# lucidrains/magvit2-pytorch

Measured on NVIDIA H100. Metric: video-frames/sec tokenize+decode, 17x128x128 bf16, higher is better.
Workload: dtype bf16

## Files before the change

### magvit2_pytorch_b200/csrc/tc_common.cuh

```cuda
#pragma once
#include "common.cuh"
#include <cuda.h>
#include <mutex>

namespace mv2 {


__device__ __forceinline__ uint32_t smem_u32(const void* p) { return (uint32_t)__cvta_generic_to_shared(p); }

__device__ __forceinline__ void mbar_init(uint32_t bar, uint32_t count) {
  asm volatile("mbarrier.init.shared::cta.b64 [%0], %1;" ::"r"(bar), "r"(count));
}
__device__ __forceinline__ void mbar_expect_tx(uint32_t bar, uint32_t bytes) {
  asm volatile("mbarrier.arrive.expect_tx.shared::cta.b64 _, [%0], %1;" ::"r"(bar), "r"(bytes) : "memory");
}
__device__ __forceinline__ void mbar_wait(uint32_t bar, uint32_t parity) {
  asm volatile(
      "{\n\t"
      ".reg .pred P1;\n\t"
      "WAIT_LOOP:\n\t"
      "mbarrier.try_wait.parity.shared::cta.b64 P1, [%0], %1, 0x989680;\n\t"
      "@P1 bra DONE;\n\t"
      "bra WAIT_LOOP;\n\t"
      "DONE:\n\t"
// ... 36 lines not shown

template <int N> __device__ __forceinline__ void setmaxnreg_dec() { asm volatile("setmaxnreg.dec.sync.aligned.u32 %0;" ::"n"(N)); }
template <int N> __device__ __forceinline__ void setmaxnreg_inc() { asm volatile("setmaxnreg.inc.sync.aligned.u32 %0;" ::"n"(N)); }
template <int N> __device__ __forceinline__ void wgmma_bf16(float (&d)[N / 2], uint64_t da, uint64_t db, uint32_t scale_d);
template <> __device__ __forceinline__ void wgmma_bf16<8>(float (&d)[4], uint64_t da, uint64_t db, uint32_t scale_d) {
  asm volatile(
      "{\n\t.reg .pred p;\n\tsetp.ne.b32 p, %6, 0;\n\t"
      "wgmma.mma_async.sync.aligned.m64n8k16.f32.bf16.bf16 {%0, %1, %2, %3}, %4, %5, p, 1, 1, 0, 0;\n\t}"
      : "+f"(d[0]), "+f"(d[1]), "+f"(d[2]), "+f"(d[3])
      : "l"(da), "l"(db), "r"(scale_d));
}
template <> __device__ __forceinline__ void wgmma_bf16<16>(float (&d)[8], uint64_t da, uint64_t db, uint32_t scale_d) {
  asm volatile(
      "{\n\t.reg .pred p;\n\tsetp.ne.b32 p, %10, 0;\n\t"
      "wgmma.mma_async.sync.aligned.m64n16k16.f32.bf16.bf16 {%0, %1, %2, %3, %4, %5, %6, %7}, %8, %9, p, 1, 1, 0, 0;\n\t}"
      : "+f"(d[0]), "+f"(d[1]), "+f"(d[2]), "+f"(d[3]), "+f"(d[4]), "+f"(d[5]), "+f"(d[6]), "+f"(d[7])
      : "l"(da), "l"(db), "r"(scale_d));
}
template <> __device__ __forceinline__ void wgmma_bf16<32>(float (&d)[16], uint64_t da, uint64_t db, uint32_t scale_d) {
  asm volatile(
      "{\n\t.reg .pred p;\n\tsetp.ne.b32 p, %18, 0;\n\t"
      "wgmma.mma_async.sync.aligned.m64n32k16.f32.bf16.bf16 {%0, %1, %2, %3, %4, %5, %6, %7, %8, %9, %10, %11, %12, %13, %14, %15}, %16, %17, p, 1, 1, 0, 0;\n\t}"
      : "+f"(d[0]), "+f"(d[1]), "+f"(d[2]), "+f"(d[3]), "+f"(d[4]), "+f"(d[5]), "+f"(d[6]), "+f"(d[7]), "+f"(d[8]), "+f"(d[9]), "+f"(d[10]), "+f"(d[11]), "+f"(d[12]), "+f"(d[13]), "+f"(d[14]), "+f"(d[15])
      : "l"(da), "l"(db), "r"(scale_d));
}
template <> __device__ __forceinline__ void wgmma_bf16<64>(float (&d)[32], uint64_t da, uint64_t db, uint32_t scale_d) {
  asm volatile(
      "{\n\t.reg .pred p;\n\tsetp.ne.b32 p, %34, 0;\n\t"
      "wgmma.mma_async.sync.aligned.m64n64k16.f32.bf16.bf16 {%0, %1, %2, %3, %4, %5, %6, %7, %8, %9, %10, %11, %12, %13, %14, %15, %16, %17, %18, %19, %20, %21, %22, %23, %24, %25, %26, %27, %28, %29, %30, %31}, %32, %33, p, 1, 1, 0, 0;\n\t}"
      : "+f"(d[0]), "+f"(d[1]), "+f"(d[2]), "+f"(d[3]), "+f"(d[4]), "+f"(d[5]), "+f"(d[6]), "+f"(d[7]), "+f"(d[8]), "+f"(d[9]), "+f"(d[10]), "+f"(d[11]), "+f"(d[12]), "+f"(d[13]), "+f"(d[14]), "+f"(d[15]), "+f"(d[16]), "+f"(d[17]), "+f"(d[18]), "+f"(d[19]), "+f"(d[20]), "+f"(d[21]), "+f"(d[22]), "+f"(d[23]), "+f"(d[24]), "+f"(d[25]), "+f"(d[26]), "+f"(d[27]), "+f"(d[28]), "+f"(d[29]), "+f"(d[30]), "+f"(d[31])
      : "l"(da), "l"(db), "r"(scale_d));
}
template <> __device__ __forceinline__ void wgmma_bf16<128>(float (&d)[64], uint64_t da, uint64_t db, uint32_t scale_d) {
  asm volatile(
      "{\n\t.reg .pred p;\n\tsetp.ne.b32 p, %66, 0;\n\t"
      "wgmma.mma_async.sync.aligned.m64n128k16.f32.bf16.bf16 {%0, %1, %2, %3, %4, %5, %6, %7, %8, %9, %10, %11, %12, %13, %14, %15, %16, %17, %18, %19, %20, %21, %22, %23, %24, %25, %26, %27, %28, %29, %30, %31, %32, %33, %34, %35, %36, %37, %38, %39, %40, %41, %42, %43, %44, %45, %46, %47, %48, %49, %50, %51, %52, %53, %54, %55, %56, %57, %58, %59, %60, %61, %62, %63}, %64, %65, p, 1, 1, 0, 0;\n\t}"
      : "+f"(d[0]), "+f"(d[1]), "+f"(d[2]), "+f"(d[3]), "+f"(d[4]), "+f"(d[5]), "+f"(d[6]), "+f"(d[7]), "+f"(d[8]), "+f"(d[9]), "+f"(d[10]), "+f"(d[11]), "+f"(d[12]), "+f"(d[13]), "+f"(d[14]), "+f"(d[15]), "+f"(d[16]), "+f"(d[17]), "+f"(d[18]), "+f"(d[19]), "+f"(d[20]), "+f"(d[21]), "+f"(d[22]), "+f"(d[23]), "+f"(d[24]), "+f"(d[25]), "+f"(d[26]), "+f"(d[27]), "+f"(d[28]), "+f"(d[29]), "+f"(d[30]), "+f"(d[31]), "+f"(d[32]), "+f"(d[33]), "+f"(d[34]), "+f"(d[35]), "+f"(d[36]), "+f"(d[37]), "+f"(d[38]), "+f"(d[39]), "+f"(d[40]), "+f"(d[41]), "+f"(d[42]), "+f"(d[43]), "+f"(d[44]), "+f"(d[45]), "+f"(d[46]), "+f"(d[47]), "+f"(d[48]), "+f"(d[49]), "+f"(d[50]), "+f"(d[51]), "+f"(d[52]), "+f"(d[53]), "+f"(d[54]), "+f"(d[55]), "+f"(d[56]), "+f"(d[57]), "+f"(d[58]), "+f"(d[59]), "+f"(d[60]), "+f"(d[61]), "+f"(d[62]), "+f"(d[63])
      : "l"(da), "l"(db), "r"(scale_d));
}

__host__ __device__ __forceinline__ uint64_t gmma_desc_hi(uint32_t sbo, uint32_t row_bytes) {
  const uint64_t layout = row_bytes == 128 ? 1 : (row_bytes == 64 ? 2 : 3);
  return ((uint64_t)1 << 16) | ((uint64_t)(sbo >> 4) << 32) | (layout << 62);
}
__device__ __forceinline__ uint32_t desc_lo(uint32_t saddr) { return (saddr & 0x3FFFF) >> 4; }

template <int N> __device__ __forceinline__ void stage_acc(const float (&d)[N / 2], float* stg, int t) {
  const int r = 16 * (t >> 5) + ((t & 31) >> 2), c = 2 * (t & 3);
#pragma unroll
  for (int j = 0; j < N / 8; ++j) {
    *reinterpret_cast<float2*>(stg + r * (N + 4) + 8 * j + c) = make_float2(d[4 * j], d[4 * j + 1]);
    *reinterpret_cast<float2*>(stg + (r + 8) * (N + 4) + 8 * j + c) = make_float2(d[4 * j + 2], d[4 * j + 3]);
  }
}
__device__ __forceinline__ void load_row32(const float* src, int ncols, uint32_t (&r)[32]) {
#pragma unroll
  for (int g = 0; g < 8; ++g) {
    if (g * 4 >= ncols) break;
    const float4 v = *reinterpret_cast<const float4*>(src + 4 * g);
    r[4 * g] = __float_as_uint(v.x); r[4 * g + 1] = __float_as_uint(v.y);
    r[4 * g + 2] = __float_as_uint(v.z); r[4 * g + 3] = __float_as_uint(v.w);
  }
}
__device__ __forceinline__ void named_bar_sync(uint32_t id, uint32_t nthreads) {
  asm volatile("bar.sync %0, %1;" ::"r"(id), "r"(nthreads) : "memory");
}
__device__ __forceinline__ void mbar_arrive(uint32_t bar) {
  asm volatile("mbarrier.arrive.shared::cta.b64 _, [%0];" ::"r"(bar) : "memory");
}

__device__ __forceinline__ uint32_t pack_bf16x2(float a, float b) {
  __nv_bfloat162 v = __floats2bfloat162_rn(a, b);
  return *reinterpret_cast<uint32_t*>(&v);
}



struct TcEpi {
  const float* bias;
  const __nv_bfloat16* res;
  __nv_bfloat16* y;
  int act, shuffle, mode;
  int Co;
  int To, Ho, Wo;
  int out_cf;
  const float* oscale;
};

__device__ __forceinline__ void store8_bf16(__nv_bfloat16* dst, const float (&v)[8]) {
  uint4 o;
  o.x = pack_bf16x2(v[0], v[1]); o.y = pack_bf16x2(v[2], v[3]);
  o.z = pack_bf16x2(v[4], v[5]); o.w = pack_bf16x2(v[6], v[7]);
  *reinterpret_cast<uint4*>(dst) = o;
}

enum { EPI_PLAIN = 0, EPI_GEGLU = 1, EPI_SHUFFLE = 2, EPI_RAGGED = 3, EPI_PLAIN_RES = 4, EPI_FUSED_RU = 5, EPI_SHUFFLE_ST = 6,
       EPI_DOWN_SPACE = 7 };

__device__ __forceinline__ float ex2_approx(float x) {
  float y;
  asm("ex2.approx.ftz.f32 %0, %1;" : "=f"(y) : "f"(x));
  return y;
}
__device__ __forceinline__ float rcp_approx(float x) {
  float y;
  asm("rcp.approx.ftz.f32 %0, %1;" : "=f"(y) : "f"(x));
// ... 189 lines not shown
```

### magvit2_pytorch_b200/csrc/tc_slab.cu

```cuda
#include "common.cuh"
#include "tc_common.cuh"
#include <cuda.h>
#include <algorithm>
#include <type_traits>
#include <mutex>
#include <map>
#include <vector>
#include <string.h>

namespace mv2 {

struct alignas(64) SlabParams {
  CUtensorMap amap;
  CUtensorMap hmap;
  CUtensorMap wmap;
  CUtensorMap wmap2;
  int kt, kh, kw, pt, ph, pw;
  int st;
  int hist_T;
  int Ci, kchunks, row_bytes;
  int B, T, H, W, Co;
  int mw, pitch, slab_h, slab_bytes, slab_stride;
  int bn, n_tiles_n, tiles_w, tiles_h, total_tiles;
  int slab_stages, w_stages;
  int tpw;
  TcEpi epi;
  CUtensorMap w1map;
  const float* bias1;
  const float* se_wk;
  float se_bk;
  float* se_ws;
  CUtensorMap amap_odd;
  int dn_e_off;
  int dn_aoff[6];
  int dn_lower;
  int h_stride;
  CUtensorMap ymap;
  CUtensorMap rmap;
};

__host__ __device__ constexpr bool slab_tma_epi(int mode) {
  return mode == EPI_PLAIN || mode == EPI_PLAIN_RES || mode == EPI_GEGLU || mode == EPI_DOWN_SPACE;
}
__host__ __device__ constexpr int slab_out_box_ch(int mode, int bn) {
  return (mode == EPI_GEGLU ? bn / 2 : bn) < 64 ? (mode == EPI_GEGLU ? bn / 2 : bn) : 64;
}

__host__ __device__ __forceinline__ void slab_frame_of(const SlabParams& p, int slot, int& b, int& t) {
  const int ptc = p.pt > 0 ? (p.pt + p.st - 1) / p.st : 0;
  const int n_cheap = ptc < p.T ? ptc : p.T, n_full = p.T - n_cheap;
  const int full_slots = p.B * n_full;
  if (slot < full_slots) { b = slot / n_full; t = n_cheap + slot - b * n_full; }
  else { const int r = slot - full_slots; const int level = r / p.B; b = r - level * p.B; t = n_cheap - 1 - level; }
}
__host__ __device__ __forceinline__ int slab_tile_of_cta(const SlabParams& p, int k, int cta, int grid) {
  const int tile = k * grid + ((k & 1) ? grid - 1 - cta : cta);
  return tile < p.total_tiles ? tile : -1;
}
__device__ __forceinline__ int slab_tile_of(const SlabParams& p, int k) { return slab_tile_of_cta(p, k, blockIdx.x, gridDim.x); }

struct TileCoord { int b, t, h0, w0, n0; };
__host__ __device__ __forceinline__ TileCoord decode_tile(const SlabParams& p, int tile) {
  TileCoord c;
  const int nt = tile % p.n_tiles_n; tile /= p.n_tiles_n;
  const int tw = tile % p.tiles_w; tile /= p.tiles_w;
  const int th = tile % p.tiles_h; tile /= p.tiles_h;
  slab_frame_of(p, tile, c.b, c.t);
  c.h0 = th * 16;
  c.w0 = tw * 8 * p.mw;
  c.n0 = nt * p.bn;
  return c;
}

struct SlabSmem { uint32_t sbias, stage0, lpart, accstg, hbuf, end, rbar, otile, rtile; };
__host__ __device__ __forceinline__ SlabSmem slab_smem_layout(const SlabParams& p, uint32_t bar0, bool fused) {
  SlabSmem m;
  m.sbias = (bar0 + 8 * (2 * p.slab_stages + 2 * p.w_stages) + 15) & ~15u;
  m.stage0 = m.sbias + (uint32_t)(p.n_tiles_n * p.bn) * 4 * (fused ? 3 : 1);
  m.lpart = m.stage0 + (fused ? 0 : 8 * 2048);
  m.accstg = m.lpart + (fused ? 2048 : 0);
  m.hbuf = m.accstg + 2u * p.mw * 64 * (p.bn + 4) * 4;
  if (fused) m.hbuf = (m.hbuf + 1023u) & ~1023u;
  m.end = m.hbuf + (fused ? (uint32_t)p.h_stride : 0);
  m.rbar = m.stage0;
  m.otile = (m.rbar + 32 + 1023u) & ~1023u;
  m.rtile = m.otile + 2u * p.mw * 64 * p.bn * 2;
  return m;
}

template <int MODE, int BN, int ACT, int MWMAX>
__device__ __forceinline__ void slab_epi_fragment(const SlabParams& p, const float (&acc)[MWMAX][BN / 2], const TileCoord& c,
                                                  const float* sbias, uint32_t ot, uint32_t rt, int wq, int lane, bool relu) {
  constexpr int OC = MODE == EPI_GEGLU ? BN / 2 : BN, CB = slab_out_box_ch(MODE, BN), NB = OC / CB;
  constexpr uint32_t RB = CB * 2, BOX = 64 * RB, SWZ = (RB / 16 - 1) << 4;
  const uint32_t m0 = 16 * wq + (lane >> 2), q4 = (lane & 3) * 4;
  auto at = [&](int j, int col, uint32_t m) {
    const uint32_t off = m * RB + (uint32_t)(col % CB) * 2 + q4;
    return (uint32_t)(j * NB + col / CB) * BOX + (off ^ ((off >> 3) & SWZ));
  };
  auto st32 = [](uint32_t a, uint32_t v) { asm volatile("st.shared.b32 [%0], %1;" ::"r"(a), "r"(v) : "memory"); };
  const float* os = (MODE == EPI_PLAIN || MODE == EPI_PLAIN_RES) && p.epi.oscale ? p.epi.oscale + (int64_t)c.b * p.Co : nullptr;
  const float rs = MODE == EPI_PLAIN_RES && p.epi.mode == 2 ? 0.70710678118654752440f : 1.f;
#pragma unroll
  for (int j = 0; j < MWMAX; ++j) {
    if (j >= p.mw) break;
    if (MODE == EPI_GEGLU) {
#pragma unroll
      for (int g = 0; g < BN / 16; ++g) {
        const int n = c.n0 + 16 * g + 2 * (lane & 3);
        const float2 bx = *reinterpret_cast<const float2*>(sbias + n), bg = *reinterpret_cast<const float2*>(sbias + n + 8);
#pragma unroll
        for (int hr = 0; hr < 2; ++hr) {
          const float* xv = &acc[j][8 * g + 2 * hr];
          const float* gv = &acc[j][8 * g + 4 + 2 * hr];
          const float v0 = gelu_fast(gv[0] + bg.x) * (xv[0] + bx.x);
          const float v1 = gelu_fast(gv[1] + bg.y) * (xv[1] + bx.y);
          st32(ot + at(j, 8 * g, m0 + 8 * hr), pack_bf16x2(v0, v1));
        }
      }
    } else {
#pragma unroll
      for (int g = 0; g < BN / 8; ++g) {
        const int col = 8 * g, n = c.n0 + col + 2 * (lane & 3);
        const float2 b = *reinterpret_cast<const float2*>(sbias + n);
        float o0 = 1.f, o1 = 1.f;
        if (os) { o0 = n < p.Co ? os[n] : 0.f; o1 = n + 1 < p.Co ? os[n + 1] : 0.f; }
#pragma unroll
        for (int hr = 0; hr < 2; ++hr) {
          float v0 = acc[j][4 * g + 2 * hr], v1 = acc[j][4 * g + 2 * hr + 1];
          if (os) { v0 *= o0; v1 *= o1; }
          v0 = act_ct<ACT>(v0 + b.x, relu);
          v1 = act_ct<ACT>(v1 + b.y, relu);
          const uint32_t a = at(j, col, m0 + 8 * hr);
          if (MODE == EPI_PLAIN_RES) {
            uint32_t r;
            asm volatile("ld.shared.b32 %0, [%1];" : "=r"(r) : "r"(rt + a) : "memory");
            v0 = (v0 + __uint_as_float(r << 16)) * rs;
            v1 = (v1 + __uint_as_float(r & 0xffff0000u)) * rs;
          }
          st32(ot + a, pack_bf16x2(v0, v1));
        }
      }
    }
  }
}

constexpr int SLAB_PRODUCER_REGS = 40, SLAB_CONSUMER_REGS = 232;
template <int MODE, int BN>
__global__ void __launch_bounds__(384, 1) tc_slab_kernel(const __grid_constant__ SlabParams p) {
  constexpr int MWMAX = BN >= 32 ? 128 / BN : 4;
  constexpr int KC1 = BN >= 64 ? BN / 64 : 1;
  extern __shared__ uint8_t smem_raw[];
  const uint32_t smem_base = (smem_u32(smem_raw) + 1023u) & ~1023u;
  const int warp = threadIdx.x >> 5, lane = threadIdx.x & 31;
  const uint32_t row_bytes = p.row_bytes;
  const uint32_t bk = row_bytes >> 1;
  const uint32_t w_tile = p.bn * row_bytes;
  const uint32_t w_bytes = w_tile * p.tpw;
  const uint32_t slab0 = smem_base;
  const uint32_t wst0 = smem_base + p.slab_stages * p.slab_stride;
  const uint32_t bar0 = wst0 + p.w_stages * w_bytes;
  const uint32_t slab_full = bar0, slab_empty = slab_full + 8 * p.slab_stages;
  const uint32_t w_full = slab_empty + 8 * p.slab_stages, w_empty = w_full + 8 * p.w_stages;
  const SlabSmem L = slab_smem_layout(p, bar0, MODE == EPI_FUSED_RU);
  auto gen = [&](uint32_t u) { return smem_raw + (u - smem_u32(smem_raw)); };
  float* sbias = reinterpret_cast<float*>(gen(L.sbias));
  const uint32_t nbias = (uint32_t)(p.n_tiles_n * p.bn);
  const uint32_t stage0 = L.stage0;

  if (threadIdx.x == 0) {
    for (int s = 0; s < p.slab_stages; ++s) { mbar_init(slab_full + 8 * s, 1); mbar_init(slab_empty + 8 * s, 8); }
    for (int s = 0; s < p.w_stages; ++s) { mbar_init(w_full + 8 * s, 1); mbar_init(w_empty + 8 * s, 8); }
    if (MODE == EPI_PLAIN_RES)
      for (int g = 0; g < 2; ++g) { mbar_init(L.rbar + 8 * g, 1); mbar_init(L.rbar + 16 + 8 * g, 4); }
    fence_barrier_init();
  }
  if (warp == 0 && lane == 0) {
    tma_prefetch_desc(&p.amap);
    if (MODE == EPI_DOWN_SPACE) tma_prefetch_desc(&p.amap_odd);
    else if (p.hist_T > 0) tma_prefetch_desc(&p.hmap);
  }
  if (warp == 2 && lane == 0) {
    tma_prefetch_desc(&p.wmap); tma_prefetch_desc(&p.wmap2);
    if (MODE == EPI_FUSED_RU) tma_prefetch_desc(&p.w1map);
  }
  if (slab_tma_epi(MODE) && warp == 1 && lane == 0) {
    tma_prefetch_desc(&p.ymap);
    if (MODE == EPI_PLAIN_RES) tma_prefetch_desc(&p.rmap);
  }
  if (warp >= 4) {
    const int nb = p.n_tiles_n * p.bn;
    for (int i = threadIdx.x - 128; i < nb; i += 256) sbias[i] = (p.epi.bias && i < p.Co) ? p.epi.bias[i] : 0.f;
    if (MODE == EPI_FUSED_RU)
      for (int i = threadIdx.x - 128; i < nb; i += 256) {
        sbias[nb + i] = (p.bias1 && i < p.Co) ? p.bias1[i] : 0.f;
        sbias[2 * nb + i] = i < p.Co ? p.se_wk[i] : 0.f;
      }
  }
  __syncthreads();
  pdl_wait();
  pdl_launch_dependents();

  const int taps2d = p.kh * p.kw;

// ... 57 lines not shown
      if (MODE == EPI_DOWN_SPACE) {
        if (lane == 0) {
          uint32_t s = 0, ph = 0;
          const int C2 = p.Ci;
          for (int tk = 0, tile; (tile = slab_tile_of(p, tk)) >= 0; ++tk) {
            const TileCoord c = decode_tile(p, tile);
            for (int kc = 0; kc < p.kchunks; ++kc)
              for (int tap = kc < p.dn_lower ? 1 : 0; tap < 6; tap += kc < p.dn_lower ? 2 : 1) {
                mbar_wait(w_empty + 8 * s, ph ^ 1);
                mbar_expect_tx(w_full + 8 * s, w_tile);
                tma_load_2d(wst0 + s * w_bytes, &p.wmap2, w_full + 8 * s, tap * C2 + kc * (int)bk, c.n0);
                if (++s == (uint32_t)p.w_stages) { s = 0; ph ^= 1; }
              }
          }
        }
      } else
      if (lane == 0) {
        uint32_t s = 0, ph = 0;
        for (int tk = 0, tile; (tile = slab_tile_of(p, tk)) >= 0; ++tk) {
          const TileCoord c = decode_tile(p, tile);
          const int dt0 = max(0, p.pt - c.t * p.st - p.hist_T);
          for (int dt = dt0; dt < p.kt; ++dt)
            for (int kc = 0; kc < p.kchunks; ++kc)
              for (int tp = 0; tp < taps2d; tp += p.tpw) {
                mbar_wait(w_empty + 8 * s, ph ^ 1);
                mbar_expect_tx(w_full + 8 * s, w_bytes);
                if (p.tpw == 1) tma_load_2d(wst0 + s * w_bytes, &p.wmap2, w_full + 8 * s, (dt * taps2d + tp) * p.Ci + kc * bk, c.n0);
                else tma_load_3d(wst0 + s * w_bytes, &p.wmap, w_full + 8 * s, kc * bk, c.n0, dt * taps2d + tp);
                if (++s == (uint32_t)p.w_stages) { s = 0; ph ^= 1; }
              }
          if (MODE == EPI_FUSED_RU)
            for (int kc2 = 0; kc2 < KC1; ++kc2) {
              mbar_wait(w_empty + 8 * s, ph ^ 1);
              mbar_expect_tx(w_full + 8 * s, w_tile);
              tma_load_2d(wst0 + s * w_bytes, &p.w1map, w_full + 8 * s, kc2 * (int)bk, 0);
              if (++s == (uint32_t)p.w_stages) { s = 0; ph ^= 1; }
            }
        }
      }
    }
  } else {
    setmaxnreg_inc<SLAB_CONSUMER_REGS>();
    const int wg = (warp - 4) >> 2, wq = warp & 3, tid = threadIdx.x & 127;
    const int sub = 2 * wg + (wq & 1), half = wq >> 1, ew = sub + 4 * half;
    const int row = sub * 32 + lane;
    const int lh = row >> 3, lw = row & 7;
    float* stg = reinterpret_cast<float*>(gen(L.accstg)) + (size_t)wg * p.mw * 64 * (BN + 4);
    const uint32_t wg_bar = 5 + wg;
    const uint32_t sbo = (uint32_t)p.pitch * row_bytes;
    const uint64_t a_hi = gmma_desc_hi(sbo, row_bytes);
    const uint64_t b_hi = gmma_desc_hi(8 * row_bytes, row_bytes);
    const bool k4 = bk == 64;
    const uint32_t a_row = row_bytes >> 4;
    const uint32_t a_wg = (uint32_t)wg * 8 * (sbo >> 4);
    const uint32_t a_next_dh = (uint32_t)(p.pitch - p.kw + 1) * a_row;
    const uint32_t a_mtile = 8 * a_row;
    const uint32_t w_tile16 = w_tile >> 4, w_stage16 = w_bytes >> 4;
    const uint32_t b_lo0 = desc_lo(wst0);
    uint32_t s_idx = 0, s_par = 0;
    uint32_t w_idx = 0, w_par = 0, b_lo = b_lo0;
    uint32_t ecount = 0;
    uint32_t r_par = 0;
    float acc[MWMAX][BN / 2];
    auto mainloop = [&](const TileCoord& c, auto mw_c, auto k4_c) {
      constexpr int MW = decltype(mw_c)::value;
      constexpr bool K4 = decltype(k4_c)::value;
      constexpr uint32_t NONE = ~0u;
      uint32_t accum = 0, pend_w = NONE, pend_s = NONE;
      auto release_pending = [&]() {
        __syncwarp();
        if (lane == 0) {
          if (pend_w != NONE) mbar_arrive(w_empty + 8 * pend_w);
          if (pend_s != NONE) mbar_arrive(slab_empty + 8 * pend_s);
        }
      };
      auto retire_previous = [&](uint32_t w_last, uint32_t s_last) {
        wgmma_wait<1>();
        release_pending();
        pend_w = w_last; pend_s = s_last;
      };
      auto next_w_stage = [&]() {
        if (++w_idx == (uint32_t)p.w_stages) { w_idx = 0; w_par ^= 1; b_lo = b_lo0; } else { b_lo += w_stage16; }
      };
      if (MODE == EPI_DOWN_SPACE) {
        for (int kc = 0; kc < p.kchunks; ++kc) {
          mbar_wait(slab_full + 8 * s_idx, s_par);
          const uint32_t a_base = desc_lo(slab0 + s_idx * p.slab_stride) + a_wg;
          const int t0 = kc < p.dn_lower ? 1 : 0, tstep = kc < p.dn_lower ? 2 : 1;
          for (int tap = t0; tap < 6; tap += tstep) {
            mbar_wait(w_full + 8 * w_idx, w_par);
            wgmma_fence();
            const uint64_t bd = b_hi | (uint64_t)b_lo;
#pragma unroll
            for (int j = 0; j < MW; ++j) {
              const uint64_t ad = a_hi | (uint64_t)(a_base + (uint32_t)p.dn_aoff[tap] + j * a_mtile);
              wgmma_bf16<BN>(acc[j], ad, bd, accum);
              wgmma_bf16<BN>(acc[j], ad + 2, bd + 2, 1u);
              wgmma_bf16<BN>(acc[j], ad + 4, bd + 4, 1u);
              wgmma_bf16<BN>(acc[j], ad + 6, bd + 6, 1u);
            }
            wgmma_commit();
            retire_previous(w_idx, tap + tstep >= 6 ? s_idx : NONE);
            accum = 1;
            next_w_stage();
          }
          if (++s_idx == (uint32_t)p.slab_stages) { s_idx = 0; s_par ^= 1; }
        }
      } else {
        const int dt0 = max(0, p.pt - c.t * p.st - p.hist_T);
        for (int dt = dt0; dt < p.kt; ++dt)
          for (int kc = 0; kc < p.kchunks; ++kc) {
            mbar_wait(slab_full + 8 * s_idx, s_par);
            uint32_t a_lo = desc_lo(slab0 + s_idx * p.slab_stride) + a_wg;
            int dw = 0;
            for (int tp0 = 0; tp0 < taps2d; tp0 += p.tpw) {
              mbar_wait(w_full + 8 * w_idx, w_par);
              const bool slab_last = tp0 + p.tpw >= taps2d;
              uint32_t b_cur = b_lo;
              for (int u = 0; u < p.tpw; ++u) {
                wgmma_fence();
                const uint64_t bd = b_hi | (uint64_t)b_cur;
#pragma unroll
                for (int j = 0; j < MW; ++j) {
                  const uint64_t ad = a_hi | (uint64_t)(a_lo + j * a_mtile);
                  wgmma_bf16<BN>(acc[j], ad, bd, accum);
                  wgmma_bf16<BN>(acc[j], ad + 2, bd + 2, 1u);
                  if (K4) {
                    wgmma_bf16<BN>(acc[j], ad + 4, bd + 4, 1u);
                    wgmma_bf16<BN>(acc[j], ad + 6, bd + 6, 1u);
                  }
                }
                wgmma_commit();
                const bool w_last = u == p.tpw - 1;
                retire_previous(w_last ? w_idx : NONE, w_last && slab_last ? s_idx : NONE);
                accum = 1;
                b_cur += w_tile16;
                if (++dw == p.kw) { dw = 0; a_lo += a_next_dh; } else { a_lo += a_row; }
              }
              next_w_stage();
            }
            if (++s_idx == (uint32_t)p.slab_stages) { s_idx = 0; s_par ^= 1; }
          }
      }
      wgmma_wait<0>();
      release_pending();
    };
    auto mainloop_k = [&](const TileCoord& c, auto mw_c) {
      if (MODE != EPI_FUSED_RU && MODE != EPI_DOWN_SPACE && !k4) mainloop(c, mw_c, std::false_type());
      else mainloop(c, mw_c, std::true_type());
    };
    for (int tk = 0, tile; (tile = slab_tile_of(p, tk)) >= 0; ++tk) {
      const TileCoord c = decode_tile(p, tile);
      if (MWMAX >= 4 && p.mw == 4) mainloop_k(c, std::integral_constant<int, (MWMAX >= 4 ? 4 : 1)>());
      else if (MWMAX >= 2 && p.mw == 2) mainloop_k(c, std::integral_constant<int, (MWMAX >= 2 ? 2 : 1)>());
      else mainloop_k(c, std::integral_constant<int, 1>());
      if (slab_tma_epi(MODE)) {
        constexpr int CB = slab_out_box_ch(MODE, BN), NB = (MODE == EPI_GEGLU ? BN / 2 : BN) / CB;
        constexpr uint32_t BOX = 64 * CB * 2;
        const uint32_t ot = L.otile + (uint32_t)(wg * p.mw * NB) * BOX, rt = L.rtile + (uint32_t)(wg * p.mw) * 64 * BN * 2;
        if (tid == 0) bulk_wait_read_all();
        named_bar_sync(wg_bar, 128);
        if (MODE == EPI_PLAIN_RES) mbar_wait(L.rbar + 8 * wg, r_par);
        const int act = p.epi.act;
        if (MODE == EPI_GEGLU || act == MV2_ACT_NONE)
          slab_epi_fragment<MODE, BN, MV2_ACT_NONE>(p, acc, c, sbias, ot, rt, wq, lane, false);
        else if (act == MV2_ACT_ELU) slab_epi_fragment<MODE, BN, MV2_ACT_ELU>(p, acc, c, sbias, ot, rt, wq, lane, false);
        else if (act == MV2_ACT_SILU) slab_epi_fragment<MODE, BN, MV2_ACT_SILU>(p, acc, c, sbias, ot, rt, wq, lane, false);
        else slab_epi_fragment<MODE, BN, MV2_ACT_LEAKY_RELU>(p, acc, c, sbias, ot, rt, wq, lane, act == MV2_ACT_RELU);
        if (MODE == EPI_PLAIN_RES) {
          __syncwarp();
          if (lane == 0) mbar_arrive(L.rbar + 16 + 8 * wg);
          r_par ^= 1;
        }
        fence_proxy_async();
        named_bar_sync(wg_bar, 128);
        if (tid == 0) {
          const int oc0 = MODE == EPI_GEGLU ? c.n0 / 2 : c.n0, oco = MODE == EPI_GEGLU ? p.Co / 2 : p.Co;
          const int h = c.h0 + 8 * wg;
          for (int j = 0; j < p.mw; ++j)
            for (int b = 0; b < NB; ++b)
              if (h < p.H && c.w0 + 8 * j < p.W && oc0 + b * CB < oco)
                tma_store_5d(&p.ymap, ot + (uint32_t)(j * NB + b) * BOX, oc0 + b * CB, c.w0 + 8 * j, h, c.t, c.b);
          bulk_commit();
        }
        continue;
      }
      named_bar_sync(wg_bar, 128);
#pragma unroll
      for (int j = 0; j < MWMAX; ++j) {
        if (j >= p.mw) break;
        stage_acc<BN>(acc[j], stg + j * 64 * (BN + 4), tid);
      }
      named_bar_sync(wg_bar, 128);
      const int h = c.h0 + lh;
      if (MODE == EPI_FUSED_RU) {
        const float* sb1 = sbias + nbias;
        const float* swk = sbias + 2 * nbias;
        float* lpart = reinterpret_cast<float*>(gen(L.lpart));
        const int64_t kstride = (int64_t)p.W * p.Co;
        const uint32_t wsw = (lane >> 1) & 3;
        const int rl = lane >> 2, piece = lane & 3;
        const int h20 = c.h0 + sub * 4;
        const int recs_per_frame = p.tiles_h * p.tiles_w * 4;
        float* rec = p.se_ws + ((int64_t)(c.b * p.T + c.t) * recs_per_frame + ((c.h0 >> 4) * p.tiles_w + c.w0 / (8 * p.mw)) * 4 + sub) * (p.Co + 2);
        float run_m = -INFINITY, run_s = 0.f, run_acc[2][8];
#pragma unroll
        for (int q = 0; q < 2; ++q)
#pragma unroll
          for (int i = 0; i < 8; ++i) run_acc[q][i] = 0.f;
        const uint64_t h_hi = gmma_desc_hi(1024, 128);
        const uint32_t h_lo = desc_lo(L.hbuf) + (uint32_t)wg * ((64 * 128) >> 4);
        uint32_t w1_slot[KC1], w1_par[KC1], w1_lo[KC1];
#pragma unroll
        for (int kc2 = 0; kc2 < KC1; ++kc2) {
          w1_slot[kc2] = w_idx; w1_par[kc2] = w_par; w1_lo[kc2] = b_lo;
          if (++w_idx == (uint32_t)p.w_stages) { w_idx = 0; w_par ^= 1; b_lo = b_lo0; } else { b_lo += w_stage16; }
        }
        for (int j = 0; j < p.mw; ++j) {
          const float* srow = stg + (j * 64 + row - 64 * wg) * (BN + 4);
          const uint32_t stg2 = smem_u32(stg + (j * 64 + (sub & 1) * 32) * (BN + 4)) + (uint32_t)half * 2048;
          const uint32_t wr = stg2 + lane * 64, rd = stg2 + rl * 64;
          const uint32_t hb = L.hbuf + (uint32_t)row * 128;
          for (int c0 = half * 32; c0 < p.bn; c0 += 64) {
            uint32_t r[32], pk[16];
            load_row32(srow + c0, 32, r);
            epi_pack32_t<MV2_ACT_ELU>(r, sbias + c0, pk);
            const uint32_t hrow = hb + (uint32_t)(c0 >> 6) * 16384;
            const uint32_t p0 = (uint32_t)(c0 & 63) >> 3;
#pragma unroll
            for (int g = 0; g < 4; ++g)
              asm volatile("st.shared.v4.b32 [%0], {%1, %2, %3, %4};" ::"r"(hrow + (((p0 + g) ^ ((uint32_t)row & 7u)) << 4)),
                           "r"(pk[4 * g]), "r"(pk[4 * g + 1]), "r"(pk[4 * g + 2]), "r"(pk[4 * g + 3]) : "memory");
          }
          fence_proxy_async();
          named_bar_sync(wg_bar, 128);
#pragma unroll
          for (int kc2 = 0; kc2 < KC1; ++kc2) mbar_wait(w_full + 8 * w1_slot[kc2], w1_par[kc2]);
          wgmma_fence();
#pragma unroll
          for (int kc2 = 0; kc2 < KC1; ++kc2) {
            const uint64_t ad = h_hi | (uint64_t)(h_lo + kc2 * (16384 >> 4)), bd = h_hi | (uint64_t)w1_lo[kc2];
            wgmma_bf16<BN>(acc[0], ad, bd, kc2 > 0 ? 1u : 0u);
            wgmma_bf16<BN>(acc[0], ad + 2, bd + 2, 1u);
            wgmma_bf16<BN>(acc[0], ad + 4, bd + 4, 1u);
            wgmma_bf16<BN>(acc[0], ad + 6, bd + 6, 1u);
          }
          wgmma_commit();
          wgmma_wait<0>();
          if (j == p.mw - 1) {
            __syncwarp();
            if (lane == 0)
#pragma unroll
              for (int kc2 = 0; kc2 < KC1; ++kc2) mbar_arrive(w_empty + 8 * w1_slot[kc2]);
          }
          stage_acc<BN>(acc[0], stg + j * 64 * (BN + 4), tid);
          named_bar_sync(wg_bar, 128);
          const int w = c.w0 + 8 * j + lw;
          const bool row_ok = h < p.H && w < p.W;
          uint32_t pk2[2][16];
          float lp = 0.f;
#pragma unroll
          for (int q = 0; q < 2; ++q) {
            const int c0 = half * 32 + 64 * q;
            if (c0 < p.bn) {
              uint32_t r[32];
              load_row32(srow + c0, 32, r);
              epi_pack32_t<MV2_ACT_ELU>(r, sb1 + c0, pk2[q]);
#pragma unroll
              for (int i = 0; i < 16; i += 2) {
                const float4 wv = *reinterpret_cast<const float4*>(swk + c0 + 2 * i);
                lp = fmaf(__uint_as_float(pk2[q][i] << 16), wv.x, lp);
                lp = fmaf(__uint_as_float(pk2[q][i] & 0xffff0000u), wv.y, lp);
                lp = fmaf(__uint_as_float(pk2[q][i + 1] << 16), wv.z, lp);
                lp = fmaf(__uint_as_float(pk2[q][i + 1] & 0xffff0000u), wv.w, lp);
              }
            }
          }
          float* lpb = lpart + (ecount & 1u) * 256;
          ++ecount;
          lpb[ew * 32 + lane] = lp;
          asm volatile("bar.sync %0, 64;" ::"r"(1 + sub) : "memory");
          float lg = lpb[sub * 32 + lane] + lpb[(sub + 4) * 32 + lane] + p.se_bk;
          lg = row_ok ? lg : -INFINITY;
          const float mx = warp_max(lg);
          const float ev = lg > -INFINITY ? ex2_approx((lg - mx) * 1.4426950408889634f) : 0.f;
          const float es = warp_sum(ev);
          float e4[4];
#pragma unroll
          for (int k = 0; k < 4; ++k) e4[k] = __shfl_sync(0xffffffffu, ev, 8 * k + rl);
          const float new_m = fmaxf(run_m, mx);
          const float ca = run_m > -INFINITY ? ex2_approx((run_m - new_m) * 1.4426950408889634f) : 0.f;
          const float cb = mx > -INFINITY ? ex2_approx((mx - new_m) * 1.4426950408889634f) : 0.f;
          run_s = fmaf(run_s, ca, es * cb);
          run_m = new_m;
// ... 288 lines not shown
  out6[0] = tile;
  if (tile >= 0) {
    const TileCoord c = decode_tile(p, tile);
    out6[1] = c.b; out6[2] = c.t; out6[3] = c.h0; out6[4] = c.w0; out6[5] = c.n0;
  }
  return MV2_OK;
}

extern "C" int mv2_tc_slab_forward(const mv2_tc_conv_args* a, const mv2_conv_hist* hist, void* stream) {
  MV2_CHECK_ARG(a && a->x && a->w && a->y);
  MV2_CHECK_ARG(!hist || (hist->T_h >= 0 && (hist->T_h == 0 || (hist->h && hist->clip_stride > 0))));
  if (!mv2_tc_slab_supported(a)) { set_error("mv2_tc_slab_forward: unsupported shape"); return MV2_E_UNSUPPORTED; }
  SlabParams p;
  if (const int rc = slab_fill_plan(a, p)) return rc;
  if (const int rc = slab_encode_maps(p, a, hist)) return rc;
  int mode = EPI_PLAIN;
  if (a->epi_mode == 1) mode = EPI_GEGLU;
  else if (a->shuffle != MV2_SHUFFLE_NONE && (a->Co / (a->shuffle == MV2_SHUFFLE_SPACE ? 4 : 2)) % 32 == 0) mode = EPI_SHUFFLE_ST;
  else if (a->shuffle != MV2_SHUFFLE_NONE) mode = EPI_SHUFFLE;
  else if (a->Co % 8 != 0) mode = EPI_RAGGED;
  else if (a->res) mode = EPI_PLAIN_RES;
  if (slab_tma_epi(mode))
    if (const int rc = slab_encode_out_maps(p, mode)) return rc;
  return slab_launch(mode, p, stream);
}


static void ru_as_conv_args(const mv2_tc_ru_args* a, mv2_tc_conv_args* c) {
  memset(c, 0, sizeof(*c));
  c->x = a->x; c->w = a->w3; c->bias = a->b3; c->res = nullptr; c->y = a->y;
  c->B = a->B; c->Ti = c->To = a->T; c->Hi = c->Ho = a->H; c->Wi = c->Wo = a->W; c->Ci = c->Co = a->C;
  c->kt = a->kt; c->kh = a->kh; c->kw = a->kw; c->st = c->sh = c->sw = 1;
  c->pt = a->kt - 1; c->ph = a->kh / 2; c->pw = a->kw / 2;
  c->act = MV2_ACT_ELU; c->shuffle = MV2_SHUFFLE_NONE; c->epi_mode = 0;
}

extern "C" int mv2_tc_ru_supported(const mv2_tc_ru_args* a) {
  if (!a) return 0;
  if (a->C != 64 && a->C != 128) return 0;
  if (a->W <= 8) return 0;
  if (a->kt < 1 || a->kt > 8 || a->kh < 1 || a->kh > 7 || a->kw < 1 || a->kw > 3) return 0;
  if ((a->kh & 1) == 0 || (a->kw & 1) == 0) return 0;
  mv2_tc_conv_args c;
  ru_as_conv_args(a, &c);
  return mv2_tc_slab_supported(&c);
}

static int ru_fill_plan(const mv2_tc_ru_args* a, SlabParams& p) {
  mv2_tc_conv_args c;
  ru_as_conv_args(a, &c);
  if (const int rc = slab_fill_plan(&c, p)) return rc;
  MV2_CHECK_ARG(p.bn == a->C && p.n_tiles_n == 1 && p.row_bytes == 128);
  p.tpw = 1;
  p.h_stride = p.kchunks * 16384;
  const int budget = slab_ring_budget(p, true);
  p.slab_stages = 2;
  p.w_stages = std::min(12, (budget - 2 * p.slab_stride) / (p.bn * p.row_bytes));
  MV2_CHECK_ARG(p.w_stages >= 2);
  p.bias1 = a->b1; p.se_wk = a->se_wk; p.se_bk = a->se_bk; p.se_ws = a->se_ws;
  return MV2_OK;
}

extern "C" int mv2_tc_ru_records(const mv2_tc_ru_args* a) {
  if (!mv2_tc_ru_supported(a)) { set_error("mv2_tc_ru_records: unsupported shape"); return MV2_E_UNSUPPORTED; }
  SlabParams p;
  if (const int rc = ru_fill_plan(a, p)) return rc;
  return p.tiles_h * p.tiles_w * 4;
}

extern "C" size_t mv2_tc_ru_workspace_bytes(const mv2_tc_ru_args* a) {
  const int recs = mv2_tc_ru_records(a);
  if (recs <= 0) return 0;
  const size_t F = (size_t)a->B * a->T;
  return (F * recs * (a->C + 2) + F * (a->C + 16)) * sizeof(float);
}

extern "C" int mv2_tc_ru_forward(const mv2_tc_ru_args* a, const mv2_conv_hist* hist, void* stream) {
  MV2_CHECK_ARG(a && a->x && a->w3 && a->w1 && a->y && a->se_wk && a->se_ws);
  MV2_CHECK_ARG(!hist || (hist->T_h >= 0 && (hist->T_h == 0 || (hist->h && hist->clip_stride > 0))));
  if (!mv2_tc_ru_supported(a)) { set_error("mv2_tc_ru_forward: unsupported shape"); return MV2_E_UNSUPPORTED; }
  SlabParams p;
  if (const int rc = ru_fill_plan(a, p)) return rc;
  mv2_tc_conv_args c;
  ru_as_conv_args(a, &c);
  if (const int rc = slab_encode_maps(p, &c, hist)) return rc;
  const cuuint64_t dims1[2] = {(cuuint64_t)a->C, (cuuint64_t)a->C};
  const cuuint64_t strides1[1] = {(cuuint64_t)a->C * 2};
  const cuuint32_t box1[2] = {64, (cuuint32_t)p.bn};
  if (const int rc = encode_bf16_map(&p.w1map, 2, a->w1, dims1, strides1, box1, CU_TENSOR_MAP_SWIZZLE_128B, "w1")) return rc;
  return slab_launch(EPI_FUSED_RU, p, stream);
}


extern "C" int mv2_tc_down_space_supported(const mv2_tc_conv_args* a) {
  if (!a) return 0;
  if (a->kt != 1 || a->kh != 3 || a->kw != 3 || a->st != 1 || a->sh != 2 || a->sw != 2) return 0;
  if (a->pt != 0 || a->ph != 1 || a->pw != 1) return 0;
  if ((a->Hi & 1) || (a->Wi & 1) || a->Ho != a->Hi / 2 || a->Wo != a->Wi / 2 || a->To != a->Ti) return 0;
  if (a->Ci % 64 != 0 || a->Co % 32 != 0 || a->Co > 4096) return 0;
  if (a->res || a->shuffle != MV2_SHUFFLE_NONE || a->epi_mode != 0 || a->out_layout != 0 || a->oscale) return 0;
  return 1;
}

extern "C" int mv2_tc_down_space_forward(const mv2_tc_conv_args* a, void* stream) {
  MV2_CHECK_ARG(a && a->x && a->w && a->y);
  if (!mv2_tc_down_space_supported(a)) { set_error("mv2_tc_down_space_forward: unsupported shape"); return MV2_E_UNSUPPORTED; }
  SlabParams p;
// ... 45 lines not shown
```

Baseline: 5293.

## Swap wgmma A/B operands for BN=64 slab conv to use wider N tiles

For the 64-channel plain and fused-residual slab convolutions, the weight tile becomes the M operand and the activation slab the N operand, so each warpgroup issues one wgmma with N=MW*64 instead of MW separate N=64 calls. The epilogue becomes a transposed stmatrix path that writes swizzled bf16 output directly, skipping the fp32 staging buffer. The fused-RU path writes the hidden activation straight into hbuf and resizes it per m-tile. This adds a new epilogue and TMA store mapping, with a risk of layout errors and more shared-memory use for hbuf.

```diff
diff --git a/magvit2_pytorch_b200/csrc/tc_common.cuh b/magvit2_pytorch_b200/csrc/tc_common.cuh
--- a/magvit2_pytorch_b200/csrc/tc_common.cuh
+++ b/magvit2_pytorch_b200/csrc/tc_common.cuh
@@ -112,6 +112,10 @@
     *reinterpret_cast<float2*>(stg + r * (N + 4) + 8 * j + c) = make_float2(d[4 * j], d[4 * j + 1]);
     *reinterpret_cast<float2*>(stg + (r + 8) * (N + 4) + 8 * j + c) = make_float2(d[4 * j + 2], d[4 * j + 3]);
   }
+}
+__device__ __forceinline__ void stmatrix_x4_trans(uint32_t addr, const uint32_t (&v)[4]) {
+  asm volatile("stmatrix.sync.aligned.m8n8.x4.trans.shared.b16 [%0], {%1, %2, %3, %4};"
+               ::"r"(addr), "r"(v[0]), "r"(v[1]), "r"(v[2]), "r"(v[3]) : "memory");
 }
 __device__ __forceinline__ void load_row32(const float* src, int ncols, uint32_t (&r)[32]) {
 #pragma unroll
diff --git a/magvit2_pytorch_b200/csrc/tc_slab.cu b/magvit2_pytorch_b200/csrc/tc_slab.cu
--- a/magvit2_pytorch_b200/csrc/tc_slab.cu
+++ b/magvit2_pytorch_b200/csrc/tc_slab.cu
@@ -45,6 +45,7 @@
 __host__ __device__ constexpr int slab_out_box_ch(int mode, int bn) {
   return (mode == EPI_GEGLU ? bn / 2 : bn) < 64 ? (mode == EPI_GEGLU ? bn / 2 : bn) : 64;
 }
+__host__ __device__ constexpr bool slab_swap_ab(int mode, int bn) { return bn == 64 && (mode == EPI_PLAIN || mode == EPI_FUSED_RU); }
 
 __host__ __device__ __forceinline__ void slab_frame_of(const SlabParams& p, int slot, int& b, int& t) {
   const int ptc = p.pt > 0 ? (p.pt + p.st - 1) / p.st : 0;
@@ -145,11 +146,41 @@
   }
 }
 
+template <int ACT>
+__device__ __forceinline__ void slab_epi_swapped(const SlabParams& p, const float (&d)[64], const TileCoord& c,
+                                                 const float* sbias, uint32_t ot, int wq, int lane, bool relu) {
+  const float* os = p.epi.oscale ? p.epi.oscale + (int64_t)c.b * p.Co : nullptr;
+  float b[2], o[2] = {1.f, 1.f};
+#pragma unroll
+  for (int k = 0; k < 2; ++k) {
+    const int n = c.n0 + 16 * wq + 8 * k + (lane >> 2);
+    b[k] = sbias[n];
+    if (os) o[k] = n < p.Co ? os[n] : 0.f;
+  }
+  const uint32_t m = lane >> 3, unit = 2 * wq + (m & 1);
+#pragma unroll
+  for (int i = 0; i < 8; ++i) {
+    if (i >= 4 * p.mw) break;
+    uint32_t v[4];
+#pragma unroll
+    for (int q = 0; q < 4; ++q) {
+      const int k = q & 1;
+      float v0 = d[8 * i + 2 * q], v1 = d[8 * i + 2 * q + 1];
+      if (os) { v0 *= o[k]; v1 *= o[k]; }
+      v[q] = pack_bf16x2(act_ct<ACT>(v0 + b[k], relu), act_ct<ACT>(v1 + b[k], relu));
+    }
+    const uint32_t row = 8 * (2 * i + (m >> 1)) + (lane & 7);
+    stmatrix_x4_trans(ot + row * 128 + ((unit ^ (row & 7)) << 4), v);
+  }
+}
+
 constexpr int SLAB_PRODUCER_REGS = 40, SLAB_CONSUMER_REGS = 232;
+constexpr uint32_t SLAB_CONSUMERS_BAR = 7;
 template <int MODE, int BN>
 __global__ void __launch_bounds__(384, 1) tc_slab_kernel(const __grid_constant__ SlabParams p) {
   constexpr int MWMAX = BN >= 32 ? 128 / BN : 4;
   constexpr int KC1 = BN >= 64 ? BN / 64 : 1;
+  constexpr bool SWAP = slab_swap_ab(MODE, BN);
   extern __shared__ uint8_t smem_raw[];
   const uint32_t smem_base = (smem_u32(smem_raw) + 1023u) & ~1023u;
   const int warp = threadIdx.x >> 5, lane = threadIdx.x & 31;
@@ -313,7 +344,7 @@
     const uint64_t b_hi = gmma_desc_hi(8 * row_bytes, row_bytes);
     const bool k4 = bk == 64;
     const uint32_t a_row = row_bytes >> 4;
-    const uint32_t a_wg = (uint32_t)wg * 8 * (sbo >> 4);
+    const uint32_t a_wg = SWAP && p.mw == 2 ? (uint32_t)wg * 8 * a_row : (uint32_t)wg * 8 * (sbo >> 4);
     const uint32_t a_next_dh = (uint32_t)(p.pitch - p.kw + 1) * a_row;
     const uint32_t a_mtile = 8 * a_row;
     const uint32_t w_tile16 = w_tile >> 4, w_stage16 = w_bytes >> 4;
@@ -381,14 +412,25 @@
               for (int u = 0; u < p.tpw; ++u) {
                 wgmma_fence();
                 const uint64_t bd = b_hi | (uint64_t)b_cur;
-#pragma unroll
-                for (int j = 0; j < MW; ++j) {
-                  const uint64_t ad = a_hi | (uint64_t)(a_lo + j * a_mtile);
-                  wgmma_bf16<BN>(acc[j], ad, bd, accum);
-                  wgmma_bf16<BN>(acc[j], ad + 2, bd + 2, 1u);
+                if constexpr (SWAP) {
+                  float (&d)[MW * 32] = *reinterpret_cast<float (*)[MW * 32]>(&acc[0][0]);
+                  const uint64_t sd = a_hi | (uint64_t)a_lo;
+                  wgmma_bf16<MW * 64>(d, bd, sd, accum);
+                  wgmma_bf16<MW * 64>(d, bd + 2, sd + 2, 1u);
                   if (K4) {
-                    wgmma_bf16<BN>(acc[j], ad + 4, bd + 4, 1u);
-                    wgmma_bf16<BN>(acc[j], ad + 6, bd + 6, 1u);
+                    wgmma_bf16<MW * 64>(d, bd + 4, sd + 4, 1u);
+                    wgmma_bf16<MW * 64>(d, bd + 6, sd + 6, 1u);
+                  }
+                } else {
+#pragma unroll
+                  for (int j = 0; j < MW; ++j) {
+                    const uint64_t ad = a_hi | (uint64_t)(a_lo + j * a_mtile);
+                    wgmma_bf16<BN>(acc[j], ad, bd, accum);
+                    wgmma_bf16<BN>(acc[j], ad + 2, bd + 2, 1u);
+                    if (K4) {
+                      wgmma_bf16<BN>(acc[j], ad + 4, bd + 4, 1u);
+                      wgmma_bf16<BN>(acc[j], ad + 6, bd + 6, 1u);
+                    }
                   }
                 }
                 wgmma_commit();
@@ -423,6 +465,13 @@
         named_bar_sync(wg_bar, 128);
         if (MODE == EPI_PLAIN_RES) mbar_wait(L.rbar + 8 * wg, r_par);
         const int act = p.epi.act;
+        if constexpr (SWAP) {
+          const float (&d)[64] = *reinterpret_cast<const float (*)[64]>(&acc[0][0]);
+          if (act == MV2_ACT_NONE) slab_epi_swapped<MV2_ACT_NONE>(p, d, c, sbias, ot, wq, lane, false);
+          else if (act == MV2_ACT_ELU) slab_epi_swapped<MV2_ACT_ELU>(p, d, c, sbias, ot, wq, lane, false);
+          else if (act == MV2_ACT_SILU) slab_epi_swapped<MV2_ACT_SILU>(p, d, c, sbias, ot, wq, lane, false);
+          else slab_epi_swapped<MV2_ACT_LEAKY_RELU>(p, d, c, sbias, ot, wq, lane, act == MV2_ACT_RELU);
+        } else
         if (MODE == EPI_GEGLU || act == MV2_ACT_NONE)
           slab_epi_fragment<MODE, BN, MV2_ACT_NONE>(p, acc, c, sbias, ot, rt, wq, lane, false);
         else if (act == MV2_ACT_ELU) slab_epi_fragment<MODE, BN, MV2_ACT_ELU>(p, acc, c, sbias, ot, rt, wq, lane, false);
@@ -437,22 +486,37 @@
         named_bar_sync(wg_bar, 128);
         if (tid == 0) {
           const int oc0 = MODE == EPI_GEGLU ? c.n0 / 2 : c.n0, oco = MODE == EPI_GEGLU ? p.Co / 2 : p.Co;
-          const int h = c.h0 + 8 * wg;
-          for (int j = 0; j < p.mw; ++j)
-            for (int b = 0; b < NB; ++b)
-              if (h < p.H && c.w0 + 8 * j < p.W && oc0 + b * CB < oco)
-                tma_store_5d(&p.ymap, ot + (uint32_t)(j * NB + b) * BOX, oc0 + b * CB, c.w0 + 8 * j, h, c.t, c.b);
+          if (SWAP && p.mw == 2) {
+            const int w = c.w0 + 8 * wg;
+            for (int j = 0; j < 2; ++j)
+              if (c.h0 + 8 * j < p.H && w < p.W && oc0 < oco)
+                tma_store_5d(&p.ymap, ot + (uint32_t)j * BOX, oc0, w, c.h0 + 8 * j, c.t, c.b);
+          } else {
+            const int h = c.h0 + 8 * wg;
+            for (int j = 0; j < p.mw; ++j)
+              for (int b = 0; b < NB; ++b)
+                if (h < p.H && c.w0 + 8 * j < p.W && oc0 + b * CB < oco)
+                  tma_store_5d(&p.ymap, ot + (uint32_t)(j * NB + b) * BOX, oc0 + b * CB, c.w0 + 8 * j, h, c.t, c.b);
+          }
           bulk_commit();
         }
         continue;
       }
-      named_bar_sync(wg_bar, 128);
-#pragma unroll
-      for (int j = 0; j < MWMAX; ++j) {
-        if (j >= p.mw) break;
-        stage_acc<BN>(acc[j], stg + j * 64 * (BN + 4), tid);
+      if constexpr (SWAP) {
+        named_bar_sync(SLAB_CONSUMERS_BAR, 256);
+        slab_epi_swapped<MV2_ACT_ELU>(p, *reinterpret_cast<const float (*)[64]>(&acc[0][0]), c, sbias,
+                                      L.hbuf + (uint32_t)(wg * p.mw) * 8192, wq, lane, false);
+        fence_proxy_async();
+        named_bar_sync(SLAB_CONSUMERS_BAR, 256);
+      } else {
+        named_bar_sync(wg_bar, 128);
+#pragma unroll
+        for (int j = 0; j < MWMAX; ++j) {
+          if (j >= p.mw) break;
+          stage_acc<BN>(acc[j], stg + j * 64 * (BN + 4), tid);
+        }
+        named_bar_sync(wg_bar, 128);
       }
-      named_bar_sync(wg_bar, 128);
       const int h = c.h0 + lh;
       if (MODE == EPI_FUSED_RU) {
         const float* sb1 = sbias + nbias;
@@ -482,25 +546,28 @@
           const uint32_t stg2 = smem_u32(stg + (j * 64 + (sub & 1) * 32) * (BN + 4)) + (uint32_t)half * 2048;
           const uint32_t wr = stg2 + lane * 64, rd = stg2 + rl * 64;
           const uint32_t hb = L.hbuf + (uint32_t)row * 128;
-          for (int c0 = half * 32; c0 < p.bn; c0 += 64) {
-            uint32_t r[32], pk[16];
-            load_row32(srow + c0, 32, r);
-            epi_pack32_t<MV2_ACT_ELU>(r, sbias + c0, pk);
-            const uint32_t hrow = hb + (uint32_t)(c0 >> 6) * 16384;
-            const uint32_t p0 = (uint32_t)(c0 & 63) >> 3;
-#pragma unroll
-            for (int g = 0; g < 4; ++g)
-              asm volatile("st.shared.v4.b32 [%0], {%1, %2, %3, %4};" ::"r"(hrow + (((p0 + g) ^ ((uint32_t)row & 7u)) << 4)),
-                           "r"(pk[4 * g]), "r"(pk[4 * g + 1]), "r"(pk[4 * g + 2]), "r"(pk[4 * g + 3]) : "memory");
-          }
-          fence_proxy_async();
-          named_bar_sync(wg_bar, 128);
+          if (!SWAP) {
+            for (int c0 = half * 32; c0 < p.bn; c0 += 64) {
+              uint32_t r[32], pk[16];
+              load_row32(srow + c0, 32, r);
+              epi_pack32_t<MV2_ACT_ELU>(r, sbias + c0, pk);
+              const uint32_t hrow = hb + (uint32_t)(c0 >> 6) * 16384;
+              const uint32_t p0 = (uint32_t)(c0 & 63) >> 3;
+#pragma unroll
+              for (int g = 0; g < 4; ++g)
+                asm volatile("st.shared.v4.b32 [%0], {%1, %2, %3, %4};" ::"r"(hrow + (((p0 + g) ^ ((uint32_t)row & 7u)) << 4)),
+                             "r"(pk[4 * g]), "r"(pk[4 * g + 1]), "r"(pk[4 * g + 2]), "r"(pk[4 * g + 3]) : "memory");
+            }
+            fence_proxy_async();
+            named_bar_sync(wg_bar, 128);
+          }
 #pragma unroll
           for (int kc2 = 0; kc2 < KC1; ++kc2) mbar_wait(w_full + 8 * w1_slot[kc2], w1_par[kc2]);
           wgmma_fence();
 #pragma unroll
           for (int kc2 = 0; kc2 < KC1; ++kc2) {
-            const uint64_t ad = h_hi | (uint64_t)(h_lo + kc2 * (16384 >> 4)), bd = h_hi | (uint64_t)w1_lo[kc2];
+            const uint64_t ad = h_hi | (uint64_t)(h_lo + (SWAP ? j : 0) * (16384 >> 4) + kc2 * (16384 >> 4)),
+                           bd = h_hi | (uint64_t)w1_lo[kc2];
             wgmma_bf16<BN>(acc[0], ad, bd, kc2 > 0 ? 1u : 0u);
             wgmma_bf16<BN>(acc[0], ad + 2, bd + 2, 1u);
             wgmma_bf16<BN>(acc[0], ad + 4, bd + 4, 1u);
@@ -895,7 +962,7 @@
   if (const int rc = slab_fill_plan(&c, p)) return rc;
   MV2_CHECK_ARG(p.bn == a->C && p.n_tiles_n == 1 && p.row_bytes == 128);
   p.tpw = 1;
-  p.h_stride = p.kchunks * 16384;
+  p.h_stride = p.kchunks * 16384 * (slab_swap_ab(EPI_FUSED_RU, p.bn) ? p.mw : 1);
   const int budget = slab_ring_budget(p, true);
   p.slab_stages = 2;
   p.w_stages = std::min(12, (budget - 2 * p.slab_stride) / (p.bn * p.row_bytes));
```

After: 5347, median of 6. Within noise of the previous version (+1.0%).
